# stephanieleroux/sitrack

Measured on AMD Instinct MI355X. Metric: particle-steps/s, higher is better.
Workload: dtype f64

## Files before the change

include/sitrk.h:

```cpp
#ifndef SITRK_H
#define SITRK_H

#include <stdint.h>

#ifdef __cplusplus
extern "C" {
#endif

#define SITRK_VERSION 100

#define SITRK_OK        0
#define SITRK_EINVAL  (-1)
#define SITRK_EINDEX  (-2)
#define SITRK_EHIP    (-3)
#define SITRK_ENOMEM  (-4)

#define SITRK_F32 0
#define SITRK_F64 1

#define SITRK_FILL (-9999.0)

typedef struct sitrk_ctx sitrk_t;

int         sitrk_version(void);
// ... 80 lines not shown
int sitrk_coast_dist_buoys(sitrk_t *h, double rmax_km, double *dist, int32_t *seg);
int sitrk_coast_kernel_ms(sitrk_t *h, float *query_ms);

int sitrk_find_cells(sitrk_t *h, int64_t n, const double *yx, const int32_t *jiT_guess,
                     int32_t *jiT_out, int8_t *found);

int sitrk_seed_init(sitrk_t *h, int64_t nP, const double *latlon, const double *yx,
                    const double *latT, const double *lonT, const double *resolkm,
                    const double *sic, int32_t *jiT_out, int8_t *keep, int8_t *why);

int sitrk_nearest_point(sitrk_t *h, int64_t nP, const double *latlon, const double *latT, const double *lonT,
                        const double *resolkm, double rd_found_km, int max_itr, int32_t *ji, double *dmin);

int sitrk_nemo_seed(sitrk_t *h, int Nj, int Ni, int khss, const int8_t *tmask, const int8_t *rmask,
                    const double *latT, const double *lonT, const double *sic, const double *latF, const double *lonF,
                    double lat0, double lon0, int64_t capacity, double *latlon, double *yx, int64_t *nT, int64_t *nF);

int sitrk_subsample_cloud(sitrk_t *h, int64_t n, const double *yx, double rd_km, int8_t *keep, int64_t *nkeep, int32_t *launches);

int sitrk_cancel_too_close(sitrk_t *h, int64_t n, const double *lat, const double *lon, const int8_t *valid, const int32_t *nrec_all,
                           const int32_t *nrec_before, double rd_km, int8_t *keep, int64_t *nkeep, int64_t *nclose);

int sitrk_nearest_buoy(sitrk_t *h, int64_t n, const double *lat, const double *lon, const int8_t *valid, double rd_km, int32_t *nn,
                       double *dmin);

int sitrk_eval_inside(sitrk_t *h, int64_t n, const double *pts, const double *quads, int8_t *inside);
int sitrk_eval_euler(sitrk_t *h, int64_t n, const double *r, const double *vel, double rdt, double *out);
int sitrk_eval_haversine(sitrk_t *h, int64_t n, const double *plat, const double *plon, const double *xlat,
                         const double *xlon, double *dist);
int sitrk_eval_intersect(sitrk_t *h, int64_t n, const double *segs, int8_t *intersect, int8_t *ccw_abc);
int sitrk_eval_crossing(sitrk_t *h, int64_t n, const double *P1, const double *P2, const int32_t *jiT, int32_t *jiT_new,
                        int32_t *codes);
int sitrk_survive_mask(sitrk_t *h, const double *sic, int8_t *mask);

int sitrk_cart2geo(sitrk_t *h, int64_t n, const double *yx, double lat0, double lon0, double *latlon);
int sitrk_geo2cart(sitrk_t *h, int64_t n, const double *latlon, double lat0, double lon0, double *yx);

int sitrk_timer_start(sitrk_t *h);
int sitrk_timer_stop(sitrk_t *h, float *ms);
int sitrk_count_alive(sitrk_t *h, int64_t *nalive);

#ifdef __cplusplus
}
#endif
#endif
```

sitrack_amd/_lib.py:

```python
import ctypes as C
import os
import subprocess

import numpy as np

_HERE = os.path.dirname(os.path.abspath(__file__))
SO_PATH = os.environ.get("SITRK_LIB_PATH") or os.path.join(_HERE, "libsitrk.so")
CSRC = os.path.join(_HERE, "csrc")

SITRK_F32, SITRK_F64 = 0, 1
SAMPLE_AFTER, SAMPLE_ENTER = 0, 1
SAMPLE_MAX_FIELDS = 8
_SAMPLE_MODES = {"after": SAMPLE_AFTER, "enter": SAMPLE_ENTER, SAMPLE_AFTER: SAMPLE_AFTER, SAMPLE_ENTER: SAMPLE_ENTER}
_SLOT_FIELDS = {"u": 0, "u_ice": 0, "v": 1, "v_ice": 1, "siconc": 2, "sic": 2, 0: 0, 1: 1, 2: 2}
FillValue = -9999.0

_vp = C.c_void_p
_i64 = C.c_int64
_int = C.c_int
_dbl = C.c_double

_SIGNATURES = {
    "sitrk_version": (_int, []),
    "sitrk_create": (_int, [C.POINTER(_vp), _int]),
# ... 31 lines not shown
    "sitrk_restore_state": (_int, [_vp, _vp, _vp]),
    "sitrk_sort_buoys": (_int, [_vp]),
    "sitrk_set_resort": (_int, [_vp, _int]),
    "sitrk_step": (_int, [_vp, _int, _int]),
    "sitrk_run": (_int, [_vp, _int, _int, _int]),
    "sitrk_run_tlerp": (_int, [_vp, _int, _int, _int, _dbl, _int, _int]),
    "sitrk_fetch": (_int, [_vp, _vp, _vp, _vp, _vp]),
    "sitrk_fetch_record": (_int, [_vp, _int, _vp, _vp, _vp]),
    "sitrk_sample_slot": (_int, [_vp, _int, _int, _int, _int, _vp]),
    "sitrk_sample_fields": (_int, [_vp, _int, _int, _int, _int, _int, _int, _int, _int, C.POINTER(_vp), _i64, _vp]),
    "sitrk_deform_cells": (_int, [_vp, _i64, _vp, _vp, _vp, _vp, _i64, _int, _vp, _dbl, _vp, _vp, C.POINTER(_i64)]),
    "sitrk_deform_mark": (_int, [_vp, _int]),
    "sitrk_deform_since_mark": (_int, [_vp, _int, _i64, _int, _vp, _vp, _vp, C.POINTER(_i64)]),
    "sitrk_deform_kernel_ms": (_int, [_vp, C.POINTER(C.c_float), C.POINTER(C.c_float)]),
    "sitrk_coast_build": (_int, [_vp, _int, _int, _vp, _vp, _vp, C.POINTER(_i64), C.POINTER(_i64)]),
    "sitrk_coast_segments": (_int, [_vp, _i64, _vp, _vp, C.POINTER(_i64)]),
    "sitrk_coast_dist": (_int, [_vp, _i64, _vp, _dbl, _vp, _vp]),
    "sitrk_coast_dist_buoys": (_int, [_vp, _dbl, _vp, _vp]),
    "sitrk_coast_kernel_ms": (_int, [_vp, C.POINTER(C.c_float)]),
    "sitrk_count_alive": (_int, [_vp, C.POINTER(_i64)]),
    "sitrk_find_cells": (_int, [_vp, _i64, _vp, _vp, _vp, _vp]),
    "sitrk_seed_init": (_int, [_vp, _i64] + [_vp] * 9),
    "sitrk_nemo_seed": (_int, [_vp, _int, _int, _int] + [_vp] * 7 + [_dbl, _dbl, _i64, _vp, _vp, C.POINTER(_i64), C.POINTER(_i64)]),
    "sitrk_subsample_cloud": (_int, [_vp, _i64, _vp, _dbl, _vp, C.POINTER(_i64), C.POINTER(C.c_int32)]),
    "sitrk_cancel_too_close": (_int, [_vp, _i64, _vp, _vp, _vp, _vp, _vp, _dbl, _vp, C.POINTER(_i64), C.POINTER(_i64)]),
    "sitrk_nearest_buoy": (_int, [_vp, _i64, _vp, _vp, _vp, _dbl, _vp, _vp]),
    "sitrk_nearest_point": (_int, [_vp, _i64, _vp, _vp, _vp, _vp, _dbl, _int, _vp, _vp]),
    "sitrk_eval_haversine": (_int, [_vp, _i64, _vp, _vp, _vp, _vp, _vp]),
    "sitrk_eval_inside": (_int, [_vp, _i64, _vp, _vp, _vp]),
    "sitrk_eval_euler": (_int, [_vp, _i64, _vp, _vp, _dbl, _vp]),
    "sitrk_eval_intersect": (_int, [_vp, _i64, _vp, _vp, _vp]),
    "sitrk_eval_crossing": (_int, [_vp, _i64, _vp, _vp, _vp, _vp, _vp]),
    "sitrk_survive_mask": (_int, [_vp, _vp, _vp]),
    "sitrk_cart2geo": (_int, [_vp, _i64, _vp, _dbl, _dbl, _vp]),
    "sitrk_geo2cart": (_int, [_vp, _i64, _vp, _dbl, _dbl, _vp]),
    "sitrk_timer_start": (_int, [_vp]),
    "sitrk_timer_stop": (_int, [_vp, C.POINTER(C.c_float)]),
}


class SitrkError(RuntimeError):
    pass


def build(force=False, verbose=False):
    cmd = ["make", "-C", CSRC] + (["-B"] if force else [])
    r = subprocess.run(cmd, capture_output=True, text=True)
    if verbose or r.returncode:
        print(r.stdout + r.stderr)
    if r.returncode:
        raise SitrkError("building libsitrk.so failed (hipcc --offload-arch=gfx950)")
    return SO_PATH


_lib = None


def _one_hip_runtime():
    import importlib.util
    import sys
    if "torch" in sys.modules or os.environ.get("SITRK_HIP_RUNTIME", "") == "system":
        return
    try:
        spec = importlib.util.find_spec("torch")
    except (ImportError, ValueError):
        return
# ... 572 lines not shown

    def eval_euler(self, r, vel, rdt=3600.):
        r = as_c(r, np.float64)
        vel = as_c(vel, np.float64, r.shape, "vel")
        out = np.empty_like(r)
        self._chk(self._L.sitrk_eval_euler(self._h, r.size, _ptr(r), _ptr(vel), float(rdt), _ptr(out)))
        return out

    def eval_intersect(self, segs):
        segs = as_c(segs, np.float64)
        n = segs.shape[0]
        segs = as_c(segs, np.float64, (n, 4, 2), "segs")
        inter = np.empty(n, dtype=np.int8)
        ccw = np.empty(n, dtype=np.int8)
        self._chk(self._L.sitrk_eval_intersect(self._h, n, _ptr(segs), _ptr(inter), _ptr(ccw)))
        return inter.astype(bool), ccw.astype(bool)

    def eval_crossing(self, P1, P2, jiT):
        P1 = as_c(P1, np.float64)
        n = P1.shape[0]
        P2 = as_c(P2, np.float64, (n, 2), "P2")
        ji = as_c(jiT, np.int32, (n, 2), "jiT")
        out = np.empty((n, 2), dtype=np.int32)
        codes = np.empty((n, 2), dtype=np.int32)
        self._chk(self._L.sitrk_eval_crossing(self._h, n, _ptr(P1), _ptr(P2), _ptr(ji), _ptr(out), _ptr(codes)))
        return out, codes[:, 0], codes[:, 1]

    def survive_mask(self, sic):
        sic = as_c(sic, np.float64, (self.Nj, self.Ni), "sic")
        out = np.empty((self.Nj, self.Ni), dtype=np.int8)
        self._chk(self._L.sitrk_survive_mask(self._h, _ptr(sic), _ptr(out)))
        return out

    def cart2geo(self, yx, lat0=70., lon0=-45.):
        yx = as_c(yx, np.float64)
        out = np.empty_like(yx)
        self._chk(self._L.sitrk_cart2geo(self._h, yx.shape[0], _ptr(yx), float(lat0), float(lon0), _ptr(out)))
        return out

    def geo2cart(self, latlon, lat0=70., lon0=-45.):
        g = as_c(latlon, np.float64)
        out = np.empty_like(g)
        self._chk(self._L.sitrk_geo2cart(self._h, g.shape[0], _ptr(g), float(lat0), float(lon0), _ptr(out)))
        return out

    def timer_start(self):
        self._chk(self._L.sitrk_timer_start(self._h))

    def timer_stop(self):
        ms = C.c_float(0)
        self._chk(self._L.sitrk_timer_stop(self._h, C.byref(ms)))
        return ms.value
```

sitrack_amd/csrc/sitrk.hip:

```cpp
#include <hip/hip_runtime.h>

#include <algorithm>
#include <cmath>
#include <cstdarg>
#include <cstdio>
#include <cstring>
#include <new>
#include <thread>
#include <type_traits>
#include <vector>

#include "sitrk_internal.h"
#include "sitrk_kernels.h"
#include "sitrk_locate.h"
#include "sitrk_seed.h"

using namespace sitrk;

static thread_local char g_create_err[512] = {0};

int sitrk::fail(sitrk_ctx *h, int code, const char *fmt, ...)
{
    char *dst = h ? h->err : g_create_err;
    va_list ap;
// ... 68 lines not shown
    e = hipStreamCreateWithFlags(&c->own_stream, hipStreamNonBlocking);
    if (e == hipSuccess) e = hipStreamCreateWithFlags(&c->copy_stream, hipStreamNonBlocking);
    if (e == hipSuccess) e = hipStreamCreateWithFlags(&c->sv_stream, hipStreamNonBlocking);
    if (e == hipSuccess) e = hipEventCreate(&c->ev0);
    if (e == hipSuccess) e = hipEventCreate(&c->ev1);
    for (int b = 0; b < sitrk_ctx::kStage && e == hipSuccess; b++) e = hipEventCreateWithFlags(&c->stage_done[b], hipEventDisableTiming);
    for (int k = 0; k < sitrk_ctx::kLaunchRing && e == hipSuccess; k++) e = hipEventCreateWithFlags(&c->launch_ev[k], hipEventDisableTiming);
    if (e == hipSuccess) e = hipEventCreateWithFlags(&c->box_ev, hipEventDisableTiming);
    if (e == hipSuccess) e = hipEventCreateWithFlags(&c->lane_fork, hipEventDisableTiming);
    if (e == hipSuccess) e = hipEventCreateWithFlags(&c->lane_join, hipEventDisableTiming);
    if (e == hipSuccess) e = hipHostMalloc((void **)&c->box_host, 4 * sizeof(int), hipHostMallocDefault);
    if (e == hipSuccess) e = hipMalloc((void **)&c->counter, 4 * sizeof(unsigned long long));
    if (e != hipSuccess) {
        int rc = fail(h, SITRK_EHIP, "sitrk_create: %s", hipGetErrorString(e));
        (void)sitrk_destroy(c);
        return rc;
    }
    c->stream = c->own_stream;
    *out = c;
    return SITRK_OK;
}

SITRK_API int sitrk_destroy(sitrk_t *h)
{
    if (!h) return SITRK_OK;
    (void)hipSetDevice(h->device);
    if (h->copy_stream) (void)hipStreamSynchronize(h->copy_stream);
    if (h->sv_stream) (void)hipStreamSynchronize(h->sv_stream);
    if (h->stream) (void)hipStreamSynchronize(h->stream);
    free_buoys(h);
    deform_release(h, true);
    coast_release(h, false, true);
    free_records(h);
    dev_free(h->geo); dev_free(h->geoF); dev_free(h->orient); dev_free(h->tmask); dev_free(h->scratch); dev_free(h->counter); dev_free(h->tlerp_theta);
    if (h->box_ev) (void)hipEventDestroy(h->box_ev);
    if (h->lane_fork) (void)hipEventDestroy(h->lane_fork);
    if (h->lane_join) (void)hipEventDestroy(h->lane_join);
    if (h->box_host) (void)hipHostFree(h->box_host);
    if (h->ev0) (void)hipEventDestroy(h->ev0);
    if (h->ev1) (void)hipEventDestroy(h->ev1);
    for (int b = 0; b < sitrk_ctx::kStage; b++) if (h->stage_done[b]) (void)hipEventDestroy(h->stage_done[b]);
    for (int k = 0; k < sitrk_ctx::kLaunchRing; k++) if (h->launch_ev[k]) (void)hipEventDestroy(h->launch_ev[k]);
    for (int k = 0; k < 4096; k++) if (h->slot_ready[k]) (void)hipEventDestroy(h->slot_ready[k]);
    for (int k = 0; k < 4096; k++) if (h->slot_sv[k]) (void)hipEventDestroy(h->slot_sv[k]);
    if (h->sv_stream) (void)hipStreamDestroy(h->sv_stream);
    if (h->copy_stream) (void)hipStreamDestroy(h->copy_stream);
    if (h->own_stream) (void)hipStreamDestroy(h->own_stream);
    delete h;
    return SITRK_OK;
}

SITRK_API int sitrk_sync(sitrk_t *h)
{
    NEED(h, "null handle");
    HIPCHK(hipStreamSynchronize(h->copy_stream));
    HIPCHK(hipStreamSynchronize(h->sv_stream));
    HIPCHK(hipStreamSynchronize(h->stream));
    return SITRK_OK;
}

SITRK_API int sitrk_set_stream(sitrk_t *h, void *hip_stream)
{
    NEED(h, "null handle");
    HIPCHK(hipStreamSynchronize(h->stream));
    h->stream = hip_stream ? (hipStream_t)hip_stream : h->own_stream;
    return SITRK_OK;
}

SITRK_API int sitrk_set_grid(sitrk_t *h, int Nj, int Ni, const double *Yf, const double *Xf, const double *Yu,
                             const double *Xu, const double *Yv, const double *Xv, const int8_t *tmask)
{
    NEED(h, "null handle");
    NEED(Yf && Xf && Yu && Xu && Yv && Xv && tmask, "sitrk_set_grid: null array");
    if (Nj < 4 || Nj > 32767 || Ni < 4 || Ni > 65535)
        return fail(h, SITRK_EINVAL, "sitrk_set_grid: grid %dx%d outside 4..32767 x 4..65535", Nj, Ni);
    if ((int64_t)Nj * Ni > ((int64_t)1 << 29))
        return fail(h, SITRK_EINVAL, "sitrk_set_grid: grid %dx%d has more than 2^29 cells", Nj, Ni);
    HIPCHK(hipSetDevice(h->device));
    HIPCHK(hipStreamSynchronize(h->copy_stream));
    HIPCHK(hipStreamSynchronize(h->sv_stream));
    HIPCHK(hipStreamSynchronize(h->stream));
    dev_free(h->geo); dev_free(h->geoF); dev_free(h->orient); dev_free(h->tmask);
    h->geo = nullptr; h->geoF = nullptr; h->orient = nullptr; h->tmask = nullptr;
    free_records(h);
    free_buoys(h);
    coast_release(h, true, false);
    const size_t n = (size_t)Nj * Ni;
    HIPCHK(dev_alloc(&h->geo, n));
    HIPCHK(dev_alloc(&h->geoF, n));
    HIPCHK(dev_alloc(&h->orient, n));
    HIPCHK(dev_alloc(&h->tmask, n));
    double *s;
    RCCHK(carve_scratch(h, [&](Carver &c) { c.take(s, 6 * n, 1); }));
    const double *src[6] = {Yf, Xf, Yu, Xu, Yv, Xv};
    for (int a = 0; a < 6; a++) HIPCHK(upload(h, s + a * n, src[a], n));
    HIPCHK(upload(h, h->tmask, tmask, n));
    hipLaunchKernelGGL(build_geo_kernel, dim3(nblocks((int64_t)n)), dim3(kBlock), 0, h->stream, n, s, s + n, s + 2 * n, s + 3 * n,
                       s + 4 * n, s + 5 * n, h->geo, h->geoF);
    HIPCHK(hipGetLastError());
    hipLaunchKernelGGL(cell_orient_kernel, dim3(nblocks((int64_t)n)), dim3(kBlock), 0, h->stream, Nj, Ni, h->geo, h->orient);
    HIPCHK(hipGetLastError());
    double mg = 0.0;
    for (size_t k = 0; k < n; k++) {
        const double ay = fabs(Yf[k]), ax = fabs(Xf[k]);
        if (!(ay <= mg)) mg = ay;
        if (!(ax <= mg)) mg = ax;
    }
    h->eps_mg = 0x1p-48 * mg;
    HIPCHK(hipStreamSynchronize(h->stream));
    h->Nj = Nj; h->Ni = Ni;
    return SITRK_OK;
}

SITRK_API int sitrk_set_params(sitrk_t *h, double rdt, int uv_strategy, double rmin_conc)
{
    NEED(h, "null handle");
    NEED(uv_strategy >= 0 && uv_strategy <= 2,
         "sitrk_set_params: uv_strategy must be 0 (cell mean), 1 (nearest U/V point) or 2 (linear interpolation, not in the reference)");
    NEED(rdt > 0.0, "sitrk_set_params: rdt must be > 0");
    if (rmin_conc != h->rmin_conc) memset(h->slot_dirty, 1, sizeof(h->slot_dirty));
    h->rdt = rdt; h->uv_strategy = uv_strategy; h->rmin_conc = rmin_conc;
    return SITRK_OK;
}

SITRK_API int sitrk_set_substeps(sitrk_t *h, int nsub)
{
    NEED(h, "null handle");
    NEED(nsub >= 1 && nsub <= 1024, "sitrk_set_substeps: nsub must be in 1..1024");
    h->nsub = nsub;
    return SITRK_OK;
}

SITRK_API int sitrk_set_tuning(sitrk_t *h, const char *knob, int value)
// ... 10 lines not shown
        return SITRK_OK;
    }
    else if (!strcmp(knob, "fuse")) {
        if (value < 1 || value > kMaxFuse) return fail(h, SITRK_EINVAL, "sitrk_set_tuning: fuse must be 1..%d", kMaxFuse);
        h->fuse = value;
        return SITRK_OK;
    }
    else if (!strcmp(knob, "sort_tile")) {
        const int tj = value >> 8, ti = value & 255;
        if (value != 0 && (tj < 1 || ti < 1)) return fail(h, SITRK_EINVAL, "sitrk_set_tuning: sort_tile = tile_j*256 + tile_i");
        h->tile_j = tj; h->tile_i = ti;
        return SITRK_OK;
    }
    else if (!strcmp(knob, "patch_kb")) {
        if (value < 0 || value > 63) return fail(h, SITRK_EINVAL, "sitrk_set_tuning: patch_kb must be 0..63");
        h->patch_kb = value;
        return SITRK_OK;
    }
    else if (!strcmp(knob, "lanes")) {
        if (value < 1 || value > 2) return fail(h, SITRK_EINVAL, "sitrk_set_tuning: lanes must be 1 or 2");
        h->lanes = value;
        return SITRK_OK;
    }
    else if (!strcmp(knob, "lane_min_wg")) {
        if (value < 1) return fail(h, SITRK_EINVAL, "sitrk_set_tuning: lane_min_wg must be >= 1");
        h->lane_min_wg = value;
        return SITRK_OK;
    }
    else if (!strcmp(knob, "xcd_group")) {
        if (value < 0 || value > 4096) return fail(h, SITRK_EINVAL, "sitrk_set_tuning: xcd_group must be 0..4096");
        h->xcd_group = value;
        return SITRK_OK;
    }
    else if (!strcmp(knob, "async_survive")) {
        h->async_survive = value != 0;
        return SITRK_OK;
    }
    else if (!strcmp(knob, "fill_threads")) {
        if (value < 1 || value > 16) return fail(h, SITRK_EINVAL, "sitrk_set_tuning: fill_threads must be 1..16");
        h->fill_threads = value;
        return SITRK_OK;
    }
    else if (!strcmp(knob, "patch_margin")) {
        if (value < 0 || value > 64) return fail(h, SITRK_EINVAL, "sitrk_set_tuning: patch_margin must be 0..64");
        h->patch_margin = value;
        return SITRK_OK;
    }
    else if (!strcmp(knob, "subsample_block")) {
        if (value < 256 || value > 256 * kSubMaxPpt || (value & (value - 1)))
            return fail(h, SITRK_EINVAL, "sitrk_set_tuning: subsample_block must be a power of two in 256..%d", 256 * kSubMaxPpt);
        h->subsample_block = value;
        return SITRK_OK;
    }
    else if (!strcmp(knob, "coast_bin")) {
        if (value < 1 || value > 64) return fail(h, SITRK_EINVAL, "sitrk_set_tuning: coast_bin must be 1..64");
        h->coast_bin = value;
        return SITRK_OK;
    }
    else if (!strcmp(knob, "locate_bruteforce")) bit = TUNE_LOCATE_BRUTEFORCE;
    else return fail(h, SITRK_EINVAL, "sitrk_set_tuning: unknown knob '%s'", knob);
    h->tune = value ? (h->tune | bit) : (h->tune & ~bit);
    return SITRK_OK;
}

static inline size_t elem_size(int dtype) { return dtype == SITRK_F64 ? 8 : 4; }

// ... 50 lines not shown
}

static int slot_wait_upload(sitrk_ctx *h, int slot)
{
    if (h->slot_pending[slot]) {
        HIPCHK(hipStreamWaitEvent(h->stream, h->slot_ready[slot], 0));
        h->slot_pending[slot] = 0;
    }
    return SITRK_OK;
}

int sitrk::slot_order_read(sitrk_ctx *h, int slot, int field, const void **field_dev)
{
    RCCHK(slot_wait_upload(h, slot));
    *field_dev = slab_of(h, slot) + (size_t)field * h->Nj * h->Ni * elem_size(h->dtype);
    return SITRK_OK;
}

static int slot_wait_sv(sitrk_ctx *h, int slot)
{
    if (h->slot_sv_pending[slot]) {
        HIPCHK(hipStreamWaitEvent(h->stream, h->slot_sv[slot], 0));
        h->slot_sv_pending[slot] = 0;
    }
    return SITRK_OK;
}

static int launch_mark(sitrk_ctx *h, const int *slots, int nslots_used)
{
    const long long seq = ++h->launch_seq;
    HIPCHK(hipEventRecord(h->launch_ev[seq % sitrk_ctx::kLaunchRing], h->stream));
    for (int k = 0; k < nslots_used; k++) h->slot_used_seq[slots[k]] = seq;
    return SITRK_OK;
}

static int launch_survive(sitrk_ctx *h, bool f64, const void *sic, int8_t *kill, uint8_t *kill9, int j0, int j1, int i0, int i1,
                          const int *slots = nullptr, int nb = 1, long long sic_stride = 0, long long kill_stride = 0,
                          hipStream_t stream = nullptr)
{
    if (!stream) stream = h->stream;
    SvBox bx;
    bx.j_lo = j0; bx.j_hi = j1; bx.v_lo = j0; bx.v_hi = j1;
    bx.cv_lo = i0; bx.cv_hi = i1;
    bx.c_lo = i0 & ~3;
    SvBatch sb;
    sb.sic_stride = sic_stride; sb.kill_stride = kill_stride;
    for (int k = 0; k < kSvMaxBatch; k++) sb.slot[k] = (slots && k < nb) ? slots[k] : 0;
    if ((h->Ni & 3) == 0 && !(h->tune & TUNE_SURVIVE_TILE)) {
        bx.c_hi = (i1 + 3) & ~3;
        const unsigned gx = (unsigned)((bx.c_hi - bx.c_lo + kSvRowsCols - 1) / kSvRowsCols);
        const dim3 g(gx, (unsigned)((j1 - j0 + 4 * kSvRowsR - 1) / (4 * kSvRowsR)), (unsigned)nb);
        if (f64)
            hipLaunchKernelGGL((survive_kill9_rows_kernel<double>), g, dim3(256), 0, stream, h->Nj, h->Ni, bx, sb, h->tmask,
                               (const double *)sic, h->rmin_conc, kill, kill9);
        else
            hipLaunchKernelGGL((survive_kill9_rows_kernel<float>), g, dim3(256), 0, stream, h->Nj, h->Ni, bx, sb, h->tmask,
                               (const float *)sic, h->rmin_conc, kill, kill9);
    } else {
        bx.c_hi = i1;
        const dim3 grid((unsigned)((bx.c_hi - bx.c_lo + kSvTC - 1) / kSvTC), (unsigned)((j1 - j0 + kSvTR - 1) / kSvTR), (unsigned)nb);
        if (f64)
            hipLaunchKernelGGL((survive_kill9_kernel<double>), grid, dim3(kSvBlock), 0, stream, h->Nj, h->Ni, bx, sb, h->tmask,
                               (const double *)sic, h->rmin_conc, kill, kill9);
        else
            hipLaunchKernelGGL((survive_kill9_kernel<float>), grid, dim3(kSvBlock), 0, stream, h->Nj, h->Ni, bx, sb, h->tmask,
                               (const float *)sic, h->rmin_conc, kill, kill9);
    }
    HIPCHK(hipGetLastError());
    return SITRK_OK;
}

static int derive_mask_box_batch(sitrk_ctx *h, const int *slots, int nb, int j0, int j1, int i0, int i1, bool on_ingest = false)
{
    const size_t n = (size_t)h->Nj * h->Ni, es = elem_size(h->dtype);
    const bool empty = (j0 >= j1 || i0 >= i1);
    if (!on_ingest) {
        for (int k = 0; k < nb; k++) {
            RCCHK(slot_wait_upload(h, slots[k]));
            RCCHK(slot_wait_sv(h, slots[k]));
        }
        if (!empty) {
            RCCHK(launch_survive(h, h->dtype == SITRK_F64, (const char *)h->slabs + 2 * n * es, nullptr, h->kill9, j0, j1, i0, i1,
                                 slots, nb, (long long)(h->slab_bytes / es), (long long)n));
            RCCHK(launch_mark(h, slots, nb));
        }
    } else if (!empty) {
        for (int k = 0; k < nb; k++) {
            const int slot = slots[k];
            if (h->slot_pending[slot]) HIPCHK(hipStreamWaitEvent(h->sv_stream, h->slot_ready[slot], 0));
            if (h->slot_used_seq[slot] >= 0)
// ... 1219 lines not shown
        c.take(d1, n); c.take(d2, n);
        c.take(dj, 2 * n); c.take(dn, 2 * n); c.take(dc, 2 * n);
    }));
    HIPCHK(upload(h, d1, P1, n));
    HIPCHK(upload(h, d2, P2, n));
    HIPCHK(upload(h, dj, jiT, 2 * n));
    CrossTab tab;
    make_cross_tab(h->Ni, tab);
    hipLaunchKernelGGL(eval_crossing_kernel, dim3(nblocks(n)), dim3(kBlock), 0, h->stream, n, h->Nj, h->Ni, h->geo, d1, d2, dj, dn,
                       codes ? dc : nullptr, tab);
    HIPCHK(hipGetLastError());
    HIPCHK(download(h, jiT_new, dn, 2 * n));
    if (codes) HIPCHK(download(h, codes, dc, 2 * n));
    HIPCHK(hipStreamSynchronize(h->stream));
    return SITRK_OK;
}

SITRK_API int sitrk_survive_mask(sitrk_t *h, const double *sic, int8_t *mask)
{
    NEED(h, "null handle");
    NEED(h->geo, "sitrk_survive_mask: call sitrk_set_grid first");
    NEED(sic && mask, "sitrk_survive_mask: null array");
    HIPCHK(hipSetDevice(h->device));
    const size_t cells = (size_t)h->Nj * h->Ni;
    double *d_sic; int8_t *d_kill; uint8_t *d_kill9;
    RCCHK(carve_scratch(h, [&](Carver &c) { c.take(d_sic, cells); c.take(d_kill, cells); c.take(d_kill9, cells); }));
    HIPCHK(upload(h, d_sic, sic, cells));
    RCCHK(launch_survive(h, true, d_sic, d_kill, d_kill9, 0, h->Nj, 0, h->Ni));
    HIPCHK(download(h, mask, d_kill, cells));
    HIPCHK(hipStreamSynchronize(h->stream));
    return SITRK_OK;
}

static int project(sitrk_ctx *h, int64_t n, const double *in, double lat0, double lon0, double *out, bool inverse)
{
    NEED(h, "null handle");
    NEED(n >= 0, "projection: n < 0");
    if (n == 0) return SITRK_OK;
    NEED(in && out, "projection: null array");
    HIPCHK(hipSetDevice(h->device));
    static_assert(sizeof(pt) == sizeof(ll), "one staging layout serves both directions");
    pt *d_in, *d_out;
    RCCHK(carve_scratch(h, [&](Carver &c) { c.take(d_in, n); c.take(d_out, n); }));
    HIPCHK(upload(h, d_in, in, n));
    ProjParams pp = make_proj(lat0, lon0);
    if (inverse) hipLaunchKernelGGL(cart2geo_kernel, dim3(nblocks(n)), dim3(kBlock), 0, h->stream, n, pp, d_in, (ll *)d_out);
    else hipLaunchKernelGGL(geo2cart_kernel, dim3(nblocks(n)), dim3(kBlock), 0, h->stream, n, pp, (const ll *)d_in, d_out);
    HIPCHK(hipGetLastError());
    HIPCHK(download(h, out, d_out, n));
    HIPCHK(hipStreamSynchronize(h->stream));
    return SITRK_OK;
}

SITRK_API int sitrk_cart2geo(sitrk_t *h, int64_t n, const double *yx, double lat0, double lon0, double *latlon)
{
    return project(h, n, yx, lat0, lon0, latlon, true);
}

SITRK_API int sitrk_geo2cart(sitrk_t *h, int64_t n, const double *latlon, double lat0, double lon0, double *yx)
{
    return project(h, n, latlon, lat0, lon0, yx, false);
}

SITRK_API int sitrk_nemo_seed(sitrk_t *h, int Nj, int Ni, int khss, const int8_t *tmask, const int8_t *rmask, const double *latT,
                              const double *lonT, const double *sic, const double *latF, const double *lonF, double lat0, double lon0,
                              int64_t capacity, double *latlon, double *yx, int64_t *nT, int64_t *nF)
// ... 74 lines not shown
```

sitrack_amd/csrc/sitrk_internal.h:

```cpp
#pragma once
#include <hip/hip_runtime.h>
#include <stdint.h>
#include <stddef.h>

#include "../../include/sitrk.h"
#include "sitrk_geom.h"

namespace sitrk {

hipError_t sort_pairs_u32(void *tmp, size_t *tmp_bytes, const uint32_t *kin, uint32_t *kout,
                          const int32_t *vin, int32_t *vout, size_t n, unsigned end_bit, hipStream_t s);

struct SubGrid {
    double ymin = 0.0, xmin = 0.0, inv_h = 0.0;
    int ny = 1, nx = 1;
};
constexpr int kSubMaxPpt = 16;
struct SubResolveArgs {
    SubGrid g;
    int64_t n = 0;
    double r2 = 0.0;
    int ppt = 4;
    const pt *yx = nullptr;
    const int32_t *perm = nullptr;
// ... 46 lines not shown

__device__ __forceinline__ bool stepped_at(BuoyState st, int64_t s, int32_t c, int jrec, bool windowed)
{
    bool in_window = true;
    if (windowed) { const int2 w = st.win[s]; in_window = (jrec >= w.x) && (jrec <= w.y); }
    return in_window && (c >= 0 || st.kill_rec[s] == jrec);
}

}

struct sitrk_ctx {
    int device = 0;
    char err[512] = {0};

    hipStream_t own_stream = nullptr;
    hipStream_t stream = nullptr;
    hipStream_t copy_stream = nullptr;
    hipStream_t sv_stream = nullptr;
    hipEvent_t ev0 = nullptr, ev1 = nullptr;

    static constexpr int kStage = 2;
    void *stage[kStage] = {nullptr, nullptr};
    size_t stage_bytes = 0;
    hipEvent_t stage_done[kStage] = {nullptr, nullptr};
    int stage_next = 0;
    int stage_rows = -1;
    int stage_cols = 0;

    int Nj = 0, Ni = 0;
    sitrk::CellGeo *geo = nullptr;
    sitrk::pt *geoF = nullptr;
    int8_t *orient = nullptr;
    int8_t *tmask = nullptr;

    double rdt = 3600.0;
    int nsub = 1;
    int uv_strategy = 1;
    double rmin_conc = 0.1;
    double eps_mg = 0.0;
    int tune = sitrk::TUNE_NT_STATE;
    int step_block = 512;
    int fuse = 32;
    int tile_j = 8, tile_i = 16;
    int patch_kb = 16;
    int xcd_group = 16;
    int patch_margin = 8;
    int lanes = 2;
    int lane_min_wg = 7168;
    hipEvent_t lane_fork = nullptr, lane_join = nullptr;
    int coast_bin = 4;
    int subsample_block = 1024;
    int fill_threads = 8;

    int nslots = 0, dtype = 0;
    size_t slab_bytes = 0;
    void *slabs = nullptr;
    uint8_t *kill9 = nullptr;
    unsigned char slot_dirty[4096] = {0};
    unsigned char slot_pending[4096] = {0};
    hipEvent_t slot_ready[4096] = {nullptr};
    hipEvent_t slot_sv[4096] = {nullptr};
    unsigned char slot_sv_pending[4096] = {0};
    int async_survive = 0;
    long long slot_used_seq[4096];
    static constexpr int kLaunchRing = 64;
    hipEvent_t launch_ev[kLaunchRing] = {nullptr};
    long long launch_seq = 0;
    int slot_row_lo[4096] = {0}, slot_row_hi[4096] = {0};
    int slot_col_lo[4096] = {0}, slot_col_hi[4096] = {0};
    int band_jmin = 0, band_jmax = -1, band_age = -1;
    int band_imin = 0, band_imax = -1;
    int *box_host = nullptr;
    hipEvent_t box_ev = nullptr;
    bool box_pending = false;
    int box_pending_age = 0;
    long long n_fused_launches = 0, n_fused_records = 0, n_step_launches = 0;
    long long n_lane_segments = 0, n_lane_launches = 0;
    double *tlerp_theta = nullptr;
    int tlerp_nsub = 0;
    double tlerp_phase = -1.0;

    int64_t nP = 0;
    bool windowed = false;
    int32_t win_first_max = 0, win_last_min = 0;
    bool rim_buoys = false;
    sitrk::BuoyState st[2];
    int cur = 0;
    uint32_t *keys[2] = {nullptr, nullptr};
    int32_t *vals[2] = {nullptr, nullptr};
    void *sort_tmp = nullptr;
    size_t sort_tmp_bytes = 0;
    int resort_every = 512;
    int steps_since_sort = 0;
    bool sorted_once = false;

// ... 83 lines not shown
```

sitrack_amd/csrc/sitrk_kernels.h:

```cpp
#pragma once
#include "sitrk_internal.h"

#pragma clang fp contract(off)

namespace sitrk {

static constexpr int kBlock = 256;

__global__ void build_geo_kernel(size_t n, const double *__restrict__ Yf, const double *__restrict__ Xf,
                                 const double *__restrict__ Yu, const double *__restrict__ Xu,
                                 const double *__restrict__ Yv, const double *__restrict__ Xv,
                                 CellGeo *__restrict__ geo, pt *__restrict__ geoF)
{
    size_t k = (size_t)blockIdx.x * blockDim.x + threadIdx.x;
    if (k >= n) return;
    CellGeo g;
    g.f = make_pt(Yf[k], Xf[k]);
    geoF[k] = g.f;
    g.u = make_pt(Yu[k], Xu[k]);
    g.v = make_pt(Yv[k], Xv[k]);
    geo[k] = g;
}

__global__ void cell_orient_kernel(int Nj, int Ni, const CellGeo *__restrict__ geo, int8_t *__restrict__ orient)
// ... 101 lines not shown
        for (int q = -1; q <= 4; q++) dv6 |= (sv_col_ok(i0 + q, Ni, bx.cv_lo, bx.cv_hi) ? 1u : 0u) << (q + 1);
        const unsigned okc = dv6 & (dv6 >> 1) & (dv6 >> 2);
        const unsigned wrm = wr_kill ? ((dv6 >> 1) & 0xfu) : 0u;
        unsigned w9 = 0;
#pragma unroll
        for (int q = 0; q < 4; q++) {
            const unsigned a = (unsigned)(R0 >> (8 * q)) & 0x010101u, b = (unsigned)(R1 >> (8 * q)) & 0x010001u,
                           c = (unsigned)(R2 >> (8 * q)) & 0x010101u;
            unsigned w = (a & 1u) | ((a >> 7) & 2u) | ((a >> 14) & 4u) | ((b & 1u) << 3) | ((b >> 12) & 16u) |
                         ((c & 1u) << 5) | ((c >> 2) & 64u) | ((c >> 9) & 128u);
            const int i = i0 + q;
            if (!(ok3 && ((okc >> q) & 1u) && i >= 1 && i <= Ni - 2)) w = 0xffu;
            w9 |= w << (8 * q);
        }
        const unsigned wk = (unsigned)(R1 >> 8);
        const size_t k = (size_t)j * Ni + i0;
        if (vec && i0 + 4 <= bx.c_hi) {
            if (kill) {
                if (wrm == 0xfu) *(unsigned *)(kill + k) = wk;
                else
                    for (int q = 0; q < 4; q++)
                        if ((wrm >> q) & 1u) kill[k + q] = (int8_t)((wk >> (8 * q)) & 0xffu);
            }
            *(unsigned *)(kill9 + k) = w9;
        } else {
            for (int q = 0; q < 4 && i0 + q < Ni && i0 + q < bx.c_hi; q++) {
                if (kill && ((wrm >> q) & 1u)) kill[k + q] = (int8_t)((wk >> (8 * q)) & 0xffu);
                kill9[k + q] = (uint8_t)((w9 >> (8 * q)) & 0xffu);
            }
        }
    }
}

static constexpr int kSvRowsR = 16;
static constexpr int kSvRowsD = 4;
static_assert((kSvRowsR + 4) % kSvRowsD == 0, "the row loop is unrolled by the prefetch depth");
static constexpr int kSvRowsCols = 62 * 4;

template <typename FT> struct Row4 { FT x, y, z, w; };

template <typename FT>
__device__ __forceinline__ Row4<FT> sv_load4(const FT *__restrict__ p)
{
    Row4<FT> r;
    if (sizeof(FT) == 4) {
        const float4 t = *(const float4 *)p;
        r.x = (FT)t.x; r.y = (FT)t.y; r.z = (FT)t.z; r.w = (FT)t.w;
    } else {
        const double2 a = *(const double2 *)p, b = *(const double2 *)(p + 2);
        r.x = (FT)a.x; r.y = (FT)a.y; r.z = (FT)b.x; r.w = (FT)b.y;
    }
    return r;
}

__device__ __forceinline__ int sv_up1(int v) { return __builtin_amdgcn_update_dpp(v, v, 0x138, 0xf, 0xf, false); }
__device__ __forceinline__ int sv_dn1(int v) { return __builtin_amdgcn_update_dpp(v, v, 0x130, 0xf, 0xf, false); }
__device__ __forceinline__ float sv_shfl_up(float v) { return __int_as_float(sv_up1(__float_as_int(v))); }
__device__ __forceinline__ float sv_shfl_dn(float v) { return __int_as_float(sv_dn1(__float_as_int(v))); }
__device__ __forceinline__ double sv_shfl_up(double v)
{
    return __hiloint2double(sv_up1(__double2hiint(v)), sv_up1(__double2loint(v)));
}
__device__ __forceinline__ double sv_shfl_dn(double v)
{
    return __hiloint2double(sv_dn1(__double2hiint(v)), sv_dn1(__double2loint(v)));
}

template <typename FT>
__global__ __launch_bounds__(256) void survive_kill9_rows_kernel(int Nj, int Ni, SvBox bx, SvBatch sb,
                                                                const int8_t *__restrict__ tmask, const FT *__restrict__ sic0,
                                                                double rmin_conc, int8_t *__restrict__ kill0, uint8_t *__restrict__ kill90)
{
    const FT *__restrict__ sic = sic0 + (size_t)sb.slot[blockIdx.z] * (size_t)sb.sic_stride;
    int8_t *__restrict__ kill = kill0 ? kill0 + (size_t)sb.slot[blockIdx.z] * (size_t)sb.kill_stride : nullptr;
    uint8_t *__restrict__ kill9 = kill90 + (size_t)sb.slot[blockIdx.z] * (size_t)sb.kill_stride;
    static_assert(sizeof(FT) == 4 || sizeof(FT) == 8, "records are binary32 or binary64");
#if !defined(__gfx9__) && !defined(__GFX9__) && defined(__HIP_DEVICE_COMPILE__)
#error "survive_kill9_rows_kernel uses the wave64 DPP row shifts of the gfx9 family (wave_shr:1 / wave_shl:1): build for gfx950"
#endif
    const int j_lo = bx.j_lo, j_hi = bx.j_hi, v_lo = bx.v_lo, v_hi = bx.v_hi;
    const int lane = (int)(threadIdx.x & 63u), wv = (int)(threadIdx.x >> 6);
    const int jr0 = j_lo + ((int)blockIdx.y * 4 + wv) * kSvRowsR;
    if (jr0 >= j_hi) return;
    const int g0 = bx.c_lo + (int)blockIdx.x * kSvRowsCols + 4 * (lane - 1);
    const bool in_cols = g0 >= 0 && g0 < Ni;
    const bool out_lane = lane >= 1 && lane <= 62 && in_cols && g0 < bx.c_hi;
    unsigned dv6 = 0;
#pragma unroll
    for (int q = -1; q <= 4; q++) dv6 |= (sv_col_ok(g0 + q, Ni, bx.cv_lo, bx.cv_hi) ? 1u : 0u) << (q + 1);
    const unsigned okc = dv6 & (dv6 >> 1) & (dv6 >> 2);
    const unsigned dvc = (dv6 >> 1) & 0xfu;
    unsigned rimc = 0;
#pragma unroll
    for (int q = 0; q < 4; q++) rimc |= ((g0 + q <= 1 || g0 + q >= Ni - 2) ? 1u : 0u) << q;
    unsigned intc = 0;
#pragma unroll
    for (int q = 0; q < 4; q++) intc |= ((g0 + q >= 1 && g0 + q <= Ni - 2) ? 1u : 0u) << q;

    const int r_first = jr0 - 2, r_last = min(jr0 + kSvRowsR, j_hi) + 1;
    Row4<FT> ring_s[kSvRowsD];
    unsigned ring_t[kSvRowsD];
    const int gload = in_cols ? g0 : 0;
    auto fetch = [&](int r, Row4<FT> &sv, unsigned &tv) {
        const int rr = min(max(r, 0), min(Nj - 1, r_last));
        const size_t k = (size_t)rr * Ni + gload;
        sv = sv_load4<FT>(sic + k);
        tv = *(const unsigned *)(tmask + k);
    };
#pragma unroll
    for (int d = 0; d < kSvRowsD; d++) fetch(r_first + d, ring_s[d], ring_t[d]);

    Row4<FT> S1 = {(FT)0, (FT)0, (FT)0, (FT)0};
    FT S1up = (FT)0, S1dn = (FT)0;
    FT S0m1 = (FT)0, S0x = (FT)0, S0y = (FT)0, S0z = (FT)0;
    unsigned T1 = 0, T1up = 0, T1dn = 0, T0sh = 0;
    unsigned K0 = 0, K1 = 0;

    for (int it = 0; it < kSvRowsR + 4; it += kSvRowsD) {
#pragma unroll
        for (int d = 0; d < kSvRowsD; d++) {
            const int r = r_first + it + d;
            const Row4<FT> S2 = ring_s[d];
            const unsigned T2 = ring_t[d];
            fetch(r + kSvRowsD, ring_s[d], ring_t[d]);
            const int jm = r - 1;
            const bool rimrow = (jm <= 1) | (jm >= Nj - 2);
            unsigned kn = 0;
            {
                const FT c1[6] = {S1up, S1.x, S1.y, S1.z, S1.w, S1dn};
                const FT c0[4] = {S0m1, S0x, S0y, S0z};
                const FT c2[4] = {S2.x, S2.y, S2.z, S2.w};
                const unsigned long long w1 = ((unsigned long long)(T1up >> 24)) | ((unsigned long long)T1 << 8) | ((unsigned long long)(T1dn & 0xffu) << 40);
#pragma unroll
                for (int q = 0; q < 4; q++) {
                    const int zmt = (int)(int8_t)(w1 >> (8 * (q + 1))) + (int)(int8_t)(w1 >> (8 * (q + 2))) + (int)(int8_t)(T2 >> (8 * q)) +
                                    (int)(int8_t)(w1 >> (8 * q)) + (int)(int8_t)(T0sh >> (8 * q));
                    const double zic = 0.2 * ((double)c1[q + 1] + (double)c1[q + 2] + (double)c2[q] + (double)c1[q] + (double)c0[q]);
                    const bool kl = rimrow | (((rimc >> q) & 1u) != 0) | (zmt < 5) | (zic < rmin_conc);
                    kn |= (kl ? 1u : 0u) << q;
                }
            }
            const unsigned kup = (unsigned)sv_up1((int)kn), kdn = (unsigned)sv_dn1((int)kn);
            const unsigned K2 = ((kup >> 3) & 1u) | (kn << 1) | ((kdn & 1u) << 5);
            const int jo = r - 2;
            if (jo >= jr0 && jo < j_hi && jo < jr0 + kSvRowsR && out_lane) {
                bool ok3 = (jo >= 1) & (jo <= Nj - 2);
#pragma unroll
                for (int dj = -1; dj <= 1; dj++) {
                    const int rr = jo + dj;
                    ok3 = ok3 & ((rr <= 1) | (rr >= Nj - 2) | ((rr - 1 >= v_lo) & (rr + 1 < v_hi)));
                }
                const bool wr_kill = (jo <= 1) | (jo >= Nj - 2) | ((jo - 1 >= v_lo) & (jo + 1 < v_hi));
                unsigned w9 = 0, wk = 0;
#pragma unroll
                for (int q = 0; q < 4; q++) {
                    unsigned w = ((K0 >> q) & 7u) | (((K1 >> q) & 1u) << 3) | (((K1 >> (q + 2)) & 1u) << 4) | (((K2 >> q) & 7u) << 5);
                    if (!(ok3 && (((intc & okc) >> q) & 1u))) w = 0xffu;
                    w9 |= w << (8 * q);
                    wk |= ((K1 >> (q + 1)) & 1u) << (8 * q);
                }
                const size_t k = (size_t)jo * Ni + g0;
                if (wr_kill && kill) {
                    if (dvc == 0xfu) *(unsigned *)(kill + k) = wk;
                    else
                        for (int q = 0; q < 4; q++)
                            if ((dvc >> q) & 1u) kill[k + q] = (int8_t)((wk >> (8 * q)) & 0xffu);
                }
                *(unsigned *)(kill9 + k) = w9;
            }
            S0m1 = S1up; S0x = S1.x; S0y = S1.y; S0z = S1.z;
            T0sh = (T1 << 8) | (T1up >> 24);
            S1 = S2; T1 = T2;
            S1up = sv_shfl_up(S2.w); S1dn = sv_shfl_dn(S2.x);
            T1up = (unsigned)sv_up1((int)T2); T1dn = (unsigned)sv_dn1((int)T2);
            K0 = K1; K1 = K2;
        }
    }
}

__global__ __launch_bounds__(kBlock) void buoy_box_kernel(int64_t n, const int32_t *__restrict__ cell, int *out)
{
    __shared__ int sm[4][kBlock / 64];
    int m0 = INT32_MIN, m1 = INT32_MIN, m2 = INT32_MIN, m3 = INT32_MIN;
    auto take = [&](int32_t c) {
        if (c >= 0) {
            const int j = cell_j(c), i = cell_i(c);
            m0 = max(m0, j); m1 = max(m1, -j); m2 = max(m2, i); m3 = max(m3, -i);
        }
    };
    const int64_t n4 = n >> 2;
    for (int64_t s = (int64_t)blockIdx.x * kBlock + threadIdx.x; s < n4; s += (int64_t)gridDim.x * kBlock) {
        const int4 c = ((const int4 *)cell)[s];
        take(c.x); take(c.y); take(c.z); take(c.w);
    }
    if (blockIdx.x == 0 && threadIdx.x < (unsigned)(n & 3)) take(cell[4 * n4 + threadIdx.x]);
    for (int off = 32; off > 0; off >>= 1) {
        m0 = max(m0, __shfl_down(m0, off)); m1 = max(m1, __shfl_down(m1, off));
        m2 = max(m2, __shfl_down(m2, off)); m3 = max(m3, __shfl_down(m3, off));
    }
    if ((threadIdx.x & 63) == 0) { const int w = threadIdx.x >> 6; sm[0][w] = m0; sm[1][w] = m1; sm[2][w] = m2; sm[3][w] = m3; }
    __syncthreads();
    if (threadIdx.x < 4) {
        int m = sm[threadIdx.x][0];
        for (int w = 1; w < kBlock / 64; w++) m = max(m, sm[threadIdx.x][w]);
        if (m > __atomic_load_n(&out[threadIdx.x], __ATOMIC_RELAXED)) atomicMax(&out[threadIdx.x], m);
    }
}
// ... 1216 lines not shown
```

Baseline: 166.3 billion.

## Precompute static tmask kill bits per grid and template survive kernel on rows/kill

Adds a one-time kernel at grid setup that packs the tmask-based (zmt<5 and rim) kill decision into one nibble byte per 4-column group. The survive_kill9 rows kernel now reads this byte instead of tmask words and drops the per-row tmask shuffles and sums. The kernel is also templated on rows per wave and on whether plain kill bytes are written, which removes a runtime branch and exposes a tuning knob. The kill9 bit packing is rewritten to use a combined word. Extra device memory and a setup launch are the costs, and the fp64-only requirement for the kill path adds a new constraint.

```diff
diff --git a/include/sitrk.h b/include/sitrk.h
--- a/include/sitrk.h
+++ b/include/sitrk.h
@@ -136,6 +136,7 @@
 int sitrk_eval_crossing(sitrk_t *h, int64_t n, const double *P1, const double *P2, const int32_t *jiT, int32_t *jiT_new,
                         int32_t *codes);
 int sitrk_survive_mask(sitrk_t *h, const double *sic, int8_t *mask);
+int sitrk_survive_bytes(sitrk_t *h, int slot, uint8_t *kill9);
 
 int sitrk_cart2geo(sitrk_t *h, int64_t n, const double *yx, double lat0, double lon0, double *latlon);
 int sitrk_geo2cart(sitrk_t *h, int64_t n, const double *latlon, double lat0, double lon0, double *yx);
diff --git a/sitrack_amd/_lib.py b/sitrack_amd/_lib.py
--- a/sitrack_amd/_lib.py
+++ b/sitrack_amd/_lib.py
@@ -87,6 +87,7 @@
     "sitrk_eval_intersect": (_int, [_vp, _i64, _vp, _vp, _vp]),
     "sitrk_eval_crossing": (_int, [_vp, _i64, _vp, _vp, _vp, _vp, _vp]),
     "sitrk_survive_mask": (_int, [_vp, _vp, _vp]),
+    "sitrk_survive_bytes": (_int, [_vp, _int, _vp]),
     "sitrk_cart2geo": (_int, [_vp, _i64, _vp, _dbl, _dbl, _vp]),
     "sitrk_geo2cart": (_int, [_vp, _i64, _vp, _dbl, _dbl, _vp]),
     "sitrk_timer_start": (_int, [_vp]),
@@ -725,6 +726,11 @@
         self._chk(self._L.sitrk_survive_mask(self._h, _ptr(sic), _ptr(out)))
         return out
 
+    def survive_bytes(self, slot):
+        out = np.empty((self.Nj, self.Ni), dtype=np.uint8)
+        self._chk(self._L.sitrk_survive_bytes(self._h, int(slot), _ptr(out)))
+        return out
+
     def cart2geo(self, yx, lat0=70., lon0=-45.):
         yx = as_c(yx, np.float64)
         out = np.empty_like(yx)
diff --git a/sitrack_amd/csrc/sitrk.hip b/sitrack_amd/csrc/sitrk.hip
--- a/sitrack_amd/csrc/sitrk.hip
+++ b/sitrack_amd/csrc/sitrk.hip
@@ -124,7 +124,7 @@
     deform_release(h, true);
     coast_release(h, false, true);
     free_records(h);
-    dev_free(h->geo); dev_free(h->geoF); dev_free(h->orient); dev_free(h->tmask); dev_free(h->scratch); dev_free(h->counter); dev_free(h->tlerp_theta);
+    dev_free(h->geo); dev_free(h->geoF); dev_free(h->orient); dev_free(h->tmask); dev_free(h->sv_static); dev_free(h->scratch); dev_free(h->counter); dev_free(h->tlerp_theta);
     if (h->box_ev) (void)hipEventDestroy(h->box_ev);
     if (h->lane_fork) (void)hipEventDestroy(h->lane_fork);
     if (h->lane_join) (void)hipEventDestroy(h->lane_join);
@@ -172,8 +172,8 @@
     HIPCHK(hipStreamSynchronize(h->copy_stream));
     HIPCHK(hipStreamSynchronize(h->sv_stream));
     HIPCHK(hipStreamSynchronize(h->stream));
-    dev_free(h->geo); dev_free(h->geoF); dev_free(h->orient); dev_free(h->tmask);
-    h->geo = nullptr; h->geoF = nullptr; h->orient = nullptr; h->tmask = nullptr;
+    dev_free(h->geo); dev_free(h->geoF); dev_free(h->orient); dev_free(h->tmask); dev_free(h->sv_static);
+    h->geo = nullptr; h->geoF = nullptr; h->orient = nullptr; h->tmask = nullptr; h->sv_static = nullptr;
     free_records(h);
     free_buoys(h);
     coast_release(h, true, false);
@@ -182,6 +182,8 @@
     HIPCHK(dev_alloc(&h->geoF, n));
     HIPCHK(dev_alloc(&h->orient, n));
     HIPCHK(dev_alloc(&h->tmask, n));
+    const int G = (Ni + 3) / 4;
+    HIPCHK(dev_alloc(&h->sv_static, (size_t)Nj * G));
     double *s;
     RCCHK(carve_scratch(h, [&](Carver &c) { c.take(s, 6 * n, 1); }));
     const double *src[6] = {Yf, Xf, Yu, Xu, Yv, Xv};
@@ -191,6 +193,8 @@
                        s + 4 * n, s + 5 * n, h->geo, h->geoF);
     HIPCHK(hipGetLastError());
     hipLaunchKernelGGL(cell_orient_kernel, dim3(nblocks((int64_t)n)), dim3(kBlock), 0, h->stream, Nj, Ni, h->geo, h->orient);
+    HIPCHK(hipGetLastError());
+    hipLaunchKernelGGL(survive_static_kernel, dim3(nblocks((int64_t)Nj * G)), dim3(kBlock), 0, h->stream, Nj, Ni, G, h->tmask, h->sv_static);
     HIPCHK(hipGetLastError());
     double mg = 0.0;
     for (size_t k = 0; k < n; k++) {
@@ -267,6 +271,11 @@
         h->xcd_group = value;
         return SITRK_OK;
     }
+    else if (!strcmp(knob, "survive_rows")) {
+        if (value != 0 && value != 16 && value != 32 && value != 64) return fail(h, SITRK_EINVAL, "sitrk_set_tuning: survive_rows must be 0, 16, 32 or 64");
+        h->survive_rows = value;
+        return SITRK_OK;
+    }
     else if (!strcmp(knob, "async_survive")) {
         h->async_survive = value != 0;
         return SITRK_OK;
@@ -383,6 +392,12 @@
     HIPCHK(hipEventRecord(h->launch_ev[seq % sitrk_ctx::kLaunchRing], h->stream));
     for (int k = 0; k < nslots_used; k++) h->slot_used_seq[slots[k]] = seq;
     return SITRK_OK;
+}
+
+static inline int sv_rows_per_wave(int nb, int rows)
+{
+    (void)nb; (void)rows;
+    return 16;
 }
 
 static int launch_survive(sitrk_ctx *h, bool f64, const void *sic, int8_t *kill, uint8_t *kill9, int j0, int j1, int i0, int i1,
@@ -400,13 +415,18 @@
     if ((h->Ni & 3) == 0 && !(h->tune & TUNE_SURVIVE_TILE)) {
         bx.c_hi = (i1 + 3) & ~3;
         const unsigned gx = (unsigned)((bx.c_hi - bx.c_lo + kSvRowsCols - 1) / kSvRowsCols);
-        const dim3 g(gx, (unsigned)((j1 - j0 + 4 * kSvRowsR - 1) / (4 * kSvRowsR)), (unsigned)nb);
-        if (f64)
-            hipLaunchKernelGGL((survive_kill9_rows_kernel<double>), g, dim3(256), 0, stream, h->Nj, h->Ni, bx, sb, h->tmask,
-                               (const double *)sic, h->rmin_conc, kill, kill9);
-        else
-            hipLaunchKernelGGL((survive_kill9_rows_kernel<float>), g, dim3(256), 0, stream, h->Nj, h->Ni, bx, sb, h->tmask,
-                               (const float *)sic, h->rmin_conc, kill, kill9);
+        const int R = h->survive_rows ? h->survive_rows : sv_rows_per_wave(nb, j1 - j0);
+        const dim3 g(gx, (unsigned)((j1 - j0 + 4 * R - 1) / (4 * R)), (unsigned)nb);
+#define SV_ROWS_LAUNCH(FT, RR, KILL) \
+        hipLaunchKernelGGL((survive_kill9_rows_kernel<FT, RR, KILL>), g, dim3(256), 0, stream, h->Nj, h->Ni, bx, sb, h->sv_static, (const FT *)sic, \
+                           h->rmin_conc, kill, kill9)
+        if (kill) {
+            NEED(f64, "launch_survive: the plain bytes are derived from fp64 input only");
+            if (R == 64) SV_ROWS_LAUNCH(double, 64, true); else if (R == 32) SV_ROWS_LAUNCH(double, 32, true); else SV_ROWS_LAUNCH(double, 16, true);
+        }
+        else if (f64) { if (R == 64) SV_ROWS_LAUNCH(double, 64, false); else if (R == 32) SV_ROWS_LAUNCH(double, 32, false); else SV_ROWS_LAUNCH(double, 16, false); }
+        else          { if (R == 64) SV_ROWS_LAUNCH(float, 64, false);  else if (R == 32) SV_ROWS_LAUNCH(float, 32, false);  else SV_ROWS_LAUNCH(float, 16, false); }
+#undef SV_ROWS_LAUNCH
     } else {
         bx.c_hi = i1;
         const dim3 grid((unsigned)((bx.c_hi - bx.c_lo + kSvTC - 1) / kSvTC), (unsigned)((j1 - j0 + kSvTR - 1) / kSvTR), (unsigned)nb);
@@ -1692,6 +1712,18 @@
     return SITRK_OK;
 }
 
+SITRK_API int sitrk_survive_bytes(sitrk_t *h, int slot, uint8_t *kill9)
+{
+    RCCHK(ingest_check(h, "sitrk_survive_bytes", slot));
+    NEED(kill9, "sitrk_survive_bytes: null array");
+    HIPCHK(hipSetDevice(h->device));
+    RCCHK(slot_make_ready(h, slot));
+    const size_t cells = (size_t)h->Nj * h->Ni;
+    HIPCHK(download(h, kill9, h->kill9 + (size_t)slot * cells, cells));
+    HIPCHK(hipStreamSynchronize(h->stream));
+    return SITRK_OK;
+}
+
 static int project(sitrk_ctx *h, int64_t n, const double *in, double lat0, double lon0, double *out, bool inverse)
 {
     NEED(h, "null handle");
diff --git a/sitrack_amd/csrc/sitrk_internal.h b/sitrack_amd/csrc/sitrk_internal.h
--- a/sitrack_amd/csrc/sitrk_internal.h
+++ b/sitrack_amd/csrc/sitrk_internal.h
@@ -102,6 +102,7 @@
     sitrk::pt *geoF = nullptr;
     int8_t *orient = nullptr;
     int8_t *tmask = nullptr;
+    uint8_t *sv_static = nullptr;
 
     double rdt = 3600.0;
     int nsub = 1;
@@ -131,6 +132,7 @@
     hipEvent_t slot_ready[4096] = {nullptr};
     hipEvent_t slot_sv[4096] = {nullptr};
     unsigned char slot_sv_pending[4096] = {0};
+    int survive_rows = 0;
     int async_survive = 0;
     long long slot_used_seq[4096];
     static constexpr int kLaunchRing = 64;
diff --git a/sitrack_amd/csrc/sitrk_kernels.h b/sitrack_amd/csrc/sitrk_kernels.h
--- a/sitrack_amd/csrc/sitrk_kernels.h
+++ b/sitrack_amd/csrc/sitrk_kernels.h
@@ -157,10 +157,29 @@
     }
 }
 
-static constexpr int kSvRowsR = 16;
 static constexpr int kSvRowsD = 4;
-static_assert((kSvRowsR + 4) % kSvRowsD == 0, "the row loop is unrolled by the prefetch depth");
 static constexpr int kSvRowsCols = 62 * 4;
+
+__global__ __launch_bounds__(kBlock) void survive_static_kernel(int Nj, int Ni, int G, const int8_t *__restrict__ tmask,
+                                                                uint8_t *__restrict__ out)
+{
+    const int64_t t = (int64_t)blockIdx.x * kBlock + threadIdx.x;
+    if (t >= (int64_t)Nj * G) return;
+    const int j = (int)(t / G), g = (int)(t - (int64_t)j * G);
+    unsigned b = 0;
+#pragma unroll
+    for (int q = 0; q < 4; q++) {
+        const int i = 4 * g + q;
+        bool kl = true;
+        if (!(j <= 1 || j >= Nj - 2 || i <= 1 || i >= Ni - 2)) {
+            const size_t k = (size_t)j * Ni + i;
+            const int zmt = (int)tmask[k] + (int)tmask[k + 1] + (int)tmask[k + Ni] + (int)tmask[k - 1] + (int)tmask[k - Ni - 1];
+            kl = zmt < 5;
+        }
+        b |= (kl ? 1u : 0u) << q;
+    }
+    out[t] = (uint8_t)b;
+}
 
 template <typename FT> struct Row4 { FT x, y, z, w; };
 
@@ -191,13 +210,14 @@
     return __hiloint2double(sv_dn1(__double2hiint(v)), sv_dn1(__double2loint(v)));
 }
 
-template <typename FT>
+template <typename FT, int R, bool KILL>
 __global__ __launch_bounds__(256) void survive_kill9_rows_kernel(int Nj, int Ni, SvBox bx, SvBatch sb,
-                                                                const int8_t *__restrict__ tmask, const FT *__restrict__ sic0,
+                                                                const uint8_t *__restrict__ stat, const FT *__restrict__ sic0,
                                                                 double rmin_conc, int8_t *__restrict__ kill0, uint8_t *__restrict__ kill90)
 {
+    static_assert((R + 4) % kSvRowsD == 0, "the row loop is unrolled by the prefetch depth");
     const FT *__restrict__ sic = sic0 + (size_t)sb.slot[blockIdx.z] * (size_t)sb.sic_stride;
-    int8_t *__restrict__ kill = kill0 ? kill0 + (size_t)sb.slot[blockIdx.z] * (size_t)sb.kill_stride : nullptr;
+    int8_t *__restrict__ kill = KILL ? kill0 + (size_t)sb.slot[blockIdx.z] * (size_t)sb.kill_stride : nullptr;
     uint8_t *__restrict__ kill9 = kill90 + (size_t)sb.slot[blockIdx.z] * (size_t)sb.kill_stride;
     static_assert(sizeof(FT) == 4 || sizeof(FT) == 8, "records are binary32 or binary64");
 #if !defined(__gfx9__) && !defined(__GFX9__) && defined(__HIP_DEVICE_COMPILE__)
@@ -205,7 +225,7 @@
 #endif
     const int j_lo = bx.j_lo, j_hi = bx.j_hi, v_lo = bx.v_lo, v_hi = bx.v_hi;
     const int lane = (int)(threadIdx.x & 63u), wv = (int)(threadIdx.x >> 6);
-    const int jr0 = j_lo + ((int)blockIdx.y * 4 + wv) * kSvRowsR;
+    const int jr0 = j_lo + ((int)blockIdx.y * 4 + wv) * R;
     if (jr0 >= j_hi) return;
     const int g0 = bx.c_lo + (int)blockIdx.x * kSvRowsCols + 4 * (lane - 1);
     const bool in_cols = g0 >= 0 && g0 < Ni;
@@ -215,22 +235,19 @@
     for (int q = -1; q <= 4; q++) dv6 |= (sv_col_ok(g0 + q, Ni, bx.cv_lo, bx.cv_hi) ? 1u : 0u) << (q + 1);
     const unsigned okc = dv6 & (dv6 >> 1) & (dv6 >> 2);
     const unsigned dvc = (dv6 >> 1) & 0xfu;
-    unsigned rimc = 0;
+    unsigned sentc = 0;
 #pragma unroll
-    for (int q = 0; q < 4; q++) rimc |= ((g0 + q <= 1 || g0 + q >= Ni - 2) ? 1u : 0u) << q;
-    unsigned intc = 0;
-#pragma unroll
-    for (int q = 0; q < 4; q++) intc |= ((g0 + q >= 1 && g0 + q <= Ni - 2) ? 1u : 0u) << q;
-
-    const int r_first = jr0 - 2, r_last = min(jr0 + kSvRowsR, j_hi) + 1;
+    for (int q = 0; q < 4; q++) sentc |= ((g0 + q >= 1 && g0 + q <= Ni - 2 && ((okc >> q) & 1u)) ? 0u : 0xffu) << (8 * q);
+
+    const int r_first = jr0 - 2, r_last = min(jr0 + R, j_hi) + 1;
     Row4<FT> ring_s[kSvRowsD];
     unsigned ring_t[kSvRowsD];
-    const int gload = in_cols ? g0 : 0;
+    const int gload = in_cols ? g0 : 0, G = Ni >> 2;
+    const unsigned outside = in_cols ? 0u : 0xfu;
     auto fetch = [&](int r, Row4<FT> &sv, unsigned &tv) {
         const int rr = min(max(r, 0), min(Nj - 1, r_last));
-        const size_t k = (size_t)rr * Ni + gload;
-        sv = sv_load4<FT>(sic + k);
-        tv = *(const unsigned *)(tmask + k);
+        sv = sv_load4<FT>(sic + ((size_t)rr * Ni + gload));
+        tv = stat[(size_t)rr * G + (gload >> 2)];
     };
 #pragma unroll
     for (int d = 0; d < kSvRowsD; d++) fetch(r_first + d, ring_s[d], ring_t[d]);
@@ -238,37 +255,31 @@
     Row4<FT> S1 = {(FT)0, (FT)0, (FT)0, (FT)0};
     FT S1up = (FT)0, S1dn = (FT)0;
     FT S0m1 = (FT)0, S0x = (FT)0, S0y = (FT)0, S0z = (FT)0;
-    unsigned T1 = 0, T1up = 0, T1dn = 0, T0sh = 0;
+    unsigned T1 = 0xfu;
     unsigned K0 = 0, K1 = 0;
 
-    for (int it = 0; it < kSvRowsR + 4; it += kSvRowsD) {
+    for (int it = 0; it < R + 4; it += kSvRowsD) {
 #pragma unroll
         for (int d = 0; d < kSvRowsD; d++) {
             const int r = r_first + it + d;
             const Row4<FT> S2 = ring_s[d];
             const unsigned T2 = ring_t[d];
             fetch(r + kSvRowsD, ring_s[d], ring_t[d]);
-            const int jm = r - 1;
-            const bool rimrow = (jm <= 1) | (jm >= Nj - 2);
-            unsigned kn = 0;
+            unsigned kn = T1 | outside;
             {
                 const FT c1[6] = {S1up, S1.x, S1.y, S1.z, S1.w, S1dn};
                 const FT c0[4] = {S0m1, S0x, S0y, S0z};
                 const FT c2[4] = {S2.x, S2.y, S2.z, S2.w};
-                const unsigned long long w1 = ((unsigned long long)(T1up >> 24)) | ((unsigned long long)T1 << 8) | ((unsigned long long)(T1dn & 0xffu) << 40);
 #pragma unroll
                 for (int q = 0; q < 4; q++) {
-                    const int zmt = (int)(int8_t)(w1 >> (8 * (q + 1))) + (int)(int8_t)(w1 >> (8 * (q + 2))) + (int)(int8_t)(T2 >> (8 * q)) +
-                                    (int)(int8_t)(w1 >> (8 * q)) + (int)(int8_t)(T0sh >> (8 * q));
                     const double zic = 0.2 * ((double)c1[q + 1] + (double)c1[q + 2] + (double)c2[q] + (double)c1[q] + (double)c0[q]);
-                    const bool kl = rimrow | (((rimc >> q) & 1u) != 0) | (zmt < 5) | (zic < rmin_conc);
-                    kn |= (kl ? 1u : 0u) << q;
+                    kn |= ((zic < rmin_conc) ? 1u : 0u) << q;
                 }
             }
             const unsigned kup = (unsigned)sv_up1((int)kn), kdn = (unsigned)sv_dn1((int)kn);
             const unsigned K2 = ((kup >> 3) & 1u) | (kn << 1) | ((kdn & 1u) << 5);
             const int jo = r - 2;
-            if (jo >= jr0 && jo < j_hi && jo < jr0 + kSvRowsR && out_lane) {
+            if (jo >= jr0 && jo < j_hi && jo < jr0 + R && out_lane) {
                 bool ok3 = (jo >= 1) & (jo <= Nj - 2);
 #pragma unroll
                 for (int dj = -1; dj <= 1; dj++) {
@@ -276,28 +287,30 @@
                     ok3 = ok3 & ((rr <= 1) | (rr >= Nj - 2) | ((rr - 1 >= v_lo) & (rr + 1 < v_hi)));
                 }
                 const bool wr_kill = (jo <= 1) | (jo >= Nj - 2) | ((jo - 1 >= v_lo) & (jo + 1 < v_hi));
-                unsigned w9 = 0, wk = 0;
+                const unsigned X = K0 | (K1 << 8) | (K2 << 16);
+                unsigned w9 = ok3 ? sentc : 0xffffffffu;
 #pragma unroll
                 for (int q = 0; q < 4; q++) {
-                    unsigned w = ((K0 >> q) & 7u) | (((K1 >> q) & 1u) << 3) | (((K1 >> (q + 2)) & 1u) << 4) | (((K2 >> q) & 7u) << 5);
-                    if (!(ok3 && (((intc & okc) >> q) & 1u))) w = 0xffu;
-                    w9 |= w << (8 * q);
-                    wk |= ((K1 >> (q + 1)) & 1u) << (8 * q);
+                    const unsigned t = X >> q;
+                    w9 |= ((t & 7u) | ((t >> 5) & 8u) | ((t >> 6) & 16u) | ((t >> 11) & 0xe0u)) << (8 * q);
                 }
                 const size_t k = (size_t)jo * Ni + g0;
-                if (wr_kill && kill) {
-                    if (dvc == 0xfu) *(unsigned *)(kill + k) = wk;
-                    else
-                        for (int q = 0; q < 4; q++)
-                            if ((dvc >> q) & 1u) kill[k + q] = (int8_t)((wk >> (8 * q)) & 0xffu);
+                if (KILL) {
+                    if (wr_kill) {
+                        unsigned wk = 0;
+#pragma unroll
+                        for (int q = 0; q < 4; q++) wk |= ((K1 >> (q + 1)) & 1u) << (8 * q);
+                        if (dvc == 0xfu) *(unsigned *)(kill + k) = wk;
+                        else
+                            for (int q = 0; q < 4; q++)
+                                if ((dvc >> q) & 1u) kill[k + q] = (int8_t)((wk >> (8 * q)) & 0xffu);
+                    }
                 }
                 *(unsigned *)(kill9 + k) = w9;
             }
             S0m1 = S1up; S0x = S1.x; S0y = S1.y; S0z = S1.z;
-            T0sh = (T1 << 8) | (T1up >> 24);
             S1 = S2; T1 = T2;
             S1up = sv_shfl_up(S2.w); S1dn = sv_shfl_dn(S2.x);
-            T1up = (unsigned)sv_up1((int)T2); T1dn = (unsigned)sv_dn1((int)T2);
             K0 = K1; K1 = K2;
         }
     }
```

Measured after the change: 166.2 billion, median of 2. About the same (-0.0%).
